# denix56/SI-Mamba

Hardware: AMD Instinct MI355X
Metric: point-clouds/sec (fwd+bwd) (higher is better)
Workload: dtype f32; 1 GPU; PointMamba classifier train step (FPS+kNN grouping, encoder, spectral SAST ordering, 12 Mamba blocks d=384 at L=1024, head, AdamW), 1024 pts -> 128 patches; global_batch=64, per_gpu_batch=64, npoints=1024, patches=128, mamba_seq_len=1024, parallelism=dp1, communicator_ranks=1, library_gemm=tuned solution table (si_mamba_amd/tuned/gemm_gfx950.csv)

## Files before the change

include/simamba.h:

```cpp
#ifndef SIMAMBA_H_
#define SIMAMBA_H_

#include <stddef.h>

#ifdef __cplusplus
extern "C" {
#endif

#define SIMAMBA_ABI_VERSION 9

#define SIMAMBA_F32  0
#define SIMAMBA_BF16 1

#define SIMAMBA_OK            0
#define SIMAMBA_E_NULLPTR    -1
#define SIMAMBA_E_SHAPE      -2
#define SIMAMBA_E_DTYPE      -3
#define SIMAMBA_E_DSTATE     -4
#define SIMAMBA_E_WIDTH      -5
#define SIMAMBA_E_WORKSPACE  -6
#define SIMAMBA_E_GROUPS     -7
#define SIMAMBA_E_ALIGN      -8
#define SIMAMBA_E_VARIANT    -9
#define SIMAMBA_E_BIAS       -10
// ... 60 lines not shown
                                  void* du, void* ddelta, float* dA, float* dB, float* dC, float* dD, void* dz,
                                  float* ddelta_bias, int batch, int dim, int seqlen, int dstate, int dt_rank,
                                  int io_dtype, long long z_bstride, long long dz_bstride, long long xdbl_bstride,
                                  long long xdbl_tstride, void* stream);
int simamba_selective_scan_dt_bwd_ex(const void* u, const void* xdbl, const void* wdt, const float* A, const float* D,
                                     const void* z, const float* delta_bias, const void* dout, const float* x_ckpt,
                                     void* du, void* ddelta, float* dA, float* dB, float* dC, float* dD, void* dz,
                                     float* ddelta_bias, int batch, int dim, int seqlen, int dstate, int dt_rank,
                                     int io_dtype, long long z_bstride, long long dz_bstride, long long xdbl_bstride,
                                     long long xdbl_tstride, int flags, float* workspace, long long workspace_floats,
                                     void* stream);

int simamba_xdt_proj_fwd(const void* x, const void* wx, const void* wdt, void* xdbl, void* delta,
                         int batch, int D, int seqlen, int S, int R, int io_dtype, long long x_bstride,
                         void* stream);
int simamba_conv_xdt_proj_fwd(const void* x, const float* cw, const float* cb, const void* wx, const void* wdt,
                              void* xconv, void* xdbl, void* delta, int batch, int D, int seqlen, int S, int R,
                              int io_dtype, long long x_bstride, void* stream);

int simamba_seq_gather_fwd(const void* in, const int* idx, void* out, int batch, int channels, int G, int L,
                           long long out_bstride, int io_dtype, void* stream);
int simamba_seq_gather_bwd(const void* dout, const int* inv, void* din, int batch, int channels, int G, int L,
                           int R, long long dout_bstride, int io_dtype, void* stream);

int simamba_causal_conv1d_fwd(const void* x, const float* w, const float* bias, void* out,
                              int batch, int dim, int seqlen, int width, int silu,
                              int io_dtype, long long x_bstride, void* stream);
int simamba_causal_conv1d_bwd(const void* x, const float* w, const float* bias,
                              const void* dout, void* dx, float* dw, float* dbias,
                              int batch, int dim, int seqlen, int width, int silu,
                              int io_dtype, long long x_bstride, long long dx_bstride, void* stream);
long long simamba_causal_conv1d_bwd_workspace_floats(int batch, int dim, int seqlen, int width, int flags);
int simamba_causal_conv1d_bwd_ex(const void* x, const float* w, const float* bias,
                                 const void* dout, void* dx, float* dw, float* dbias,
                                 int batch, int dim, int seqlen, int width, int silu,
                                 int io_dtype, long long x_bstride, long long dx_bstride, int flags,
                                 float* workspace, long long workspace_floats, void* stream);

int simamba_add_layer_norm_grid(int batch, int rows_per_batch);
int simamba_add_layer_norm_fwd(const void* hidden, const float* residual, const float* rowscale,
                               const float* weight, const float* bias, float* residual_out,
                               void* normed, float* mean, float* rstd, int batch, int rows_per_batch,
                               int dim, float eps, int hidden_dtype, int out_dtype, void* stream);
int simamba_add_layer_norm_bwd(const void* dnormed, const float* dresidual_out,
                               const float* residual_out, const float* mean, const float* rstd,
                               const float* weight, const float* rowscale, float* dresidual,
// ... 37 lines not shown
                           float eps, float* mean, float* invstd, double* count, int C, void* stream);
int simamba_bn_relu_apply(const void* x, const float* gterm, int group, const float* weight, const float* bias,
                          const float* mean, const float* invstd, void* y, long long rows, int C, long long ld,
                          int io_dtype, void* stream);
int simamba_bn_relu_bwd_sums(const void* dy, const void* x, const float* gterm, int group, const float* weight,
                             const float* bias, const float* mean, const float* invstd, float* dweight,
                             float* dbias, float* partial, long long rows, int C, long long ld, int io_dtype,
                             void* stream);
int simamba_bn_relu_bwd_dx(const void* dy, const void* x, const float* gterm, int group, const float* weight,
                           const float* bias, const float* mean, const float* invstd, const float* sum_dweight,
                           const float* sum_dbias, const double* count, void* dx, float* dgterm, int dgroup,
                           long long rows, int C, long long ld, int io_dtype, void* stream);
int simamba_group_max_fwd(const void* x, void* out, unsigned char* idx, long long groups, int n, int C,
                          int io_dtype, void* stream);
int simamba_group_max_bwd(const void* dout, const unsigned char* idx, void* dx, long long groups, int n, int C,
                          int io_dtype, void* stream);

int simamba_max_linear_bwd_slabs(long long groups, int c_in);
int simamba_max_linear_bwd_dx(const void* dout, const unsigned char* idx, const void* weight, void* dx,
                              long long groups, int n, int c_in, int c_out, int io_dtype, void* stream);
int simamba_max_linear_bwd_dw(const void* dout, const unsigned char* idx, const void* x, float* dw, float* partial,
                              long long groups, int n, int c_in, int c_out, int io_dtype, void* stream);

int simamba_three_nn(const float* xyz1, const float* xyz2, int* idx, float* weight, int batch, int N, int S,
                     void* stream);
int simamba_three_interpolate_fwd(const void* feats, const int* idx, const float* weight, void* out, int batch,
                                  int N, int S, int C, int io_dtype, void* stream);
int simamba_three_interpolate_bwd(const void* dout, const int* idx, const float* weight, float* dfeats, int batch,
                                  int N, int S, int C, int io_dtype, void* stream);

int simamba_chamfer_fwd(const float* pred, const float* gt, float* dist, unsigned char* idx1, unsigned char* idx2,
                        long long pairs, int n, int m, void* stream);
int simamba_chamfer_bwd(const float* pred, const float* gt, const float* ddist, const unsigned char* idx1,
                        const unsigned char* idx2, float* dpred, long long pairs, int n, int m, void* stream);

int simamba_chamfer_large_fwd(const float* x, const float* y, float* dist, int* idx1, int* idx2, float* d1, float* d2,
                              long long pairs, int n, int m, void* stream);
int simamba_chamfer_large_bwd(const float* x, const float* y, const float* ddist, const int* idx1, const int* idx2,
                              float* dx, float* dy, long long pairs, int n, int m, void* stream);
int simamba_chamfer_large_fwd_ex(const float* x, const float* y, float* dist, int* idx1, int* idx2, float* d1,
                                 float* d2, long long pairs, int n, int m, int queries, void* stream);
int simamba_chamfer_large_bwd_ex(const float* x, const float* y, const float* ddist, const int* idx1, const int* idx2,
                                 float* dx, float* dy, long long pairs, int n, int m, int queries, void* stream);

int simamba_knn_group(const float* points, const float* centers, long long* idx, int batch, int N, int G, int K,
                      void* stream);
// ... 41 lines not shown
```

si_mamba_amd/_lib.py:

```python
from __future__ import annotations

import ctypes
import os
from ctypes import c_char_p, c_float, c_int, c_longlong, c_size_t, c_uint, c_void_p

_HERE = os.path.dirname(os.path.abspath(__file__))
LIB_PATH = os.path.join(_HERE, "libsimamba_hip.so")

F32, BF16 = 0, 1

SPEC_SYMMETRIC = 0x01
SPEC_SELF_LOOP = 0x02
SPEC_BINARY = 0x04
SPEC_MATRIX_SYM = 0x08
SPEC_SMALLEST = 0x10
SPEC_SIGMA_MEAN = 0x20
SPEC_LARGE_G = 0x40
SPEC_MAX_G = 128
SPEC_MAX_G_LARGE = 512

SCAN_AUTO, SCAN_ROWSCAN, SCAN_LPC2, SCAN_LPC4, SCAN_MIX = 0, 1, 2, 4, 6
CKPT_ROW, CKPT_SEQ = 128, 16
BWD_DETERMINISTIC = 1
NORM_RMS = 1
# ... 18 lines not shown
                                           c_int, c_int, c_int, c_int, c_int, c_int,
                                           _LL, _LL, _LL, _LL, _LL, c_int, _P]),
    "simamba_scan_bwd_workspace_floats": (_LL, [c_int, c_int, c_int, c_int, c_int, c_int]),
    "simamba_selective_scan_bwd_ex": (c_int, [_P, _P, _P, _P, _P, _P, _P, _P, _P, _P,
                                              _P, _P, _P, _P, _P, _P, _P, _P,
                                              c_int, c_int, c_int, c_int, c_int, c_int,
                                              _LL, _LL, _LL, _LL, _LL, c_int, c_int, _P, _LL, _P]),
    "simamba_selective_scan_dt_fwd": (c_int, [_P, _P, _P, _P, _P, _P, _P, _P, _P, _P,
                                              c_int, c_int, c_int, c_int, c_int, c_int,
                                              _LL, _LL, _LL, c_int, c_int, _P]),
    "simamba_selective_scan_dt_bwd": (c_int, [_P, _P, _P, _P, _P, _P, _P, _P, _P,
                                              _P, _P, _P, _P, _P, _P, _P, _P,
                                              c_int, c_int, c_int, c_int, c_int, c_int,
                                              _LL, _LL, _LL, _LL, _P]),
    "simamba_selective_scan_dt_bwd_ex": (c_int, [_P, _P, _P, _P, _P, _P, _P, _P, _P,
                                                 _P, _P, _P, _P, _P, _P, _P, _P,
                                                 c_int, c_int, c_int, c_int, c_int, c_int,
                                                 _LL, _LL, _LL, _LL, c_int, _P, _LL, _P]),
    "simamba_xdt_proj_fwd": (c_int, [_P, _P, _P, _P, _P, c_int, c_int, c_int, c_int, c_int, c_int, _LL, _P]),
    "simamba_conv_xdt_proj_fwd": (c_int, [_P, _P, _P, _P, _P, _P, _P, _P, c_int, c_int, c_int, c_int, c_int, c_int, _LL,
                                          _P]),
    "simamba_seq_gather_fwd": (c_int, [_P, _P, _P, c_int, c_int, c_int, c_int, _LL, c_int, _P]),
    "simamba_seq_gather_bwd": (c_int, [_P, _P, _P, c_int, c_int, c_int, c_int, c_int, _LL, c_int, _P]),
    "simamba_causal_conv1d_fwd": (c_int, [_P, _P, _P, _P, c_int, c_int, c_int, c_int, c_int, c_int, _LL, _P]),
    "simamba_causal_conv1d_bwd": (c_int, [_P, _P, _P, _P, _P, _P, _P,
                                          c_int, c_int, c_int, c_int, c_int, c_int, _LL, _LL, _P]),
    "simamba_causal_conv1d_bwd_workspace_floats": (_LL, [c_int, c_int, c_int, c_int, c_int]),
    "simamba_causal_conv1d_bwd_ex": (c_int, [_P, _P, _P, _P, _P, _P, _P,
                                             c_int, c_int, c_int, c_int, c_int, c_int, _LL, _LL, c_int, _P, _LL, _P]),
    "simamba_add_layer_norm_grid": (c_int, [c_int, c_int]),
    "simamba_add_layer_norm_fwd": (c_int, [_P, _P, _P, _P, _P, _P, _P, _P, _P, c_int, c_int, c_int, c_float,
                                           c_int, c_int, _P]),
    "simamba_add_layer_norm_bwd": (c_int, [_P, _P, _P, _P, _P, _P, _P, _P, _P, _P, c_int, c_int, c_int,
                                           c_int, c_int, _P]),
    "simamba_add_layer_norm_fwd_ex": (c_int, [_P, _P, _P, _P, _P, _P, _P, _P, _P, c_int, c_int, c_int, c_float,
                                              c_int, c_int, c_int, _P]),
    "simamba_add_layer_norm_bwd_ex": (c_int, [_P, _P, _P, _P, _P, _P, _P, _P, _P, _P, c_int, c_int, c_int,
                                              c_int, c_int, c_int, _P]),
    "simamba_out_proj_add_ln_fwd": (c_int, [_P, _P, _P, _P, _P, _P, _P, _P, _P, _P, c_int, c_int, c_int, c_int, c_float,
                                            c_int, _P]),
    "simamba_out_proj_add_ln_fwd_ex": (c_int, [_P, _P, _P, _P, _P, _P, _P, _P, _P, _P, c_int, c_int, c_int, c_int,
                                               c_float, c_int, c_int, _P]),
    "simamba_in_proj_fwd": (c_int, [_P, _P, _P, c_int, c_int, c_int, c_int, c_int, _P]),
    "simamba_bn_relu_grid": (c_int, [_LL]),
    "simamba_bn_relu_fwd": (c_int, [_P, _P, c_int, _P, _P, _P, _P, c_float, c_float, c_int, _P, _P, _P, _P, _LL, c_int,
                                    _LL, c_int, _P]),
    "simamba_bn_relu_bwd": (c_int, [_P, _P, _P, c_int, _P, _P, _P, _P, _P, _P, c_int, _P, _P, _P, _LL, c_int, _LL,
                                    c_int, c_int, _P]),
    "simamba_bn_stats_local": (c_int, [_P, _P, c_int, _P, _LL, _P, _LL, c_int, _LL, c_int, _P]),
    "simamba_bn_stats_merge": (c_int, [_P, c_int, _P, _P, c_float, c_float, _P, _P, _P, c_int, _P]),
    "simamba_bn_relu_apply": (c_int, [_P, _P, c_int, _P, _P, _P, _P, _P, _LL, c_int, _LL, c_int, _P]),
    "simamba_bn_relu_bwd_sums": (c_int, [_P, _P, _P, c_int, _P, _P, _P, _P, _P, _P, _P, _LL, c_int, _LL, c_int, _P]),
    "simamba_bn_relu_bwd_dx": (c_int, [_P, _P, _P, c_int, _P, _P, _P, _P, _P, _P, _P, _P, _P, c_int, _LL, c_int, _LL,
                                       c_int, _P]),
    "simamba_group_max_fwd": (c_int, [_P, _P, _P, _LL, c_int, c_int, c_int, _P]),
    "simamba_group_max_bwd": (c_int, [_P, _P, _P, _LL, c_int, c_int, c_int, _P]),
    "simamba_max_linear_bwd_slabs": (c_int, [_LL, c_int]),
    "simamba_max_linear_bwd_dx": (c_int, [_P, _P, _P, _P, _LL, c_int, c_int, c_int, c_int, _P]),
    "simamba_max_linear_bwd_dw": (c_int, [_P, _P, _P, _P, _P, _LL, c_int, c_int, c_int, c_int, _P]),
    "simamba_three_nn": (c_int, [_P, _P, _P, _P, c_int, c_int, c_int, _P]),
    "simamba_three_interpolate_fwd": (c_int, [_P, _P, _P, _P, c_int, c_int, c_int, c_int, c_int, _P]),
    "simamba_three_interpolate_bwd": (c_int, [_P, _P, _P, _P, c_int, c_int, c_int, c_int, c_int, _P]),
    "simamba_chamfer_fwd": (c_int, [_P, _P, _P, _P, _P, _LL, c_int, c_int, _P]),
    "simamba_chamfer_bwd": (c_int, [_P, _P, _P, _P, _P, _P, _LL, c_int, c_int, _P]),
    "simamba_chamfer_large_fwd": (c_int, [_P, _P, _P, _P, _P, _P, _P, _LL, c_int, c_int, _P]),
    "simamba_chamfer_large_bwd": (c_int, [_P, _P, _P, _P, _P, _P, _P, _LL, c_int, c_int, _P]),
    "simamba_chamfer_large_fwd_ex": (c_int, [_P, _P, _P, _P, _P, _P, _P, _LL, c_int, c_int, c_int, _P]),
    "simamba_chamfer_large_bwd_ex": (c_int, [_P, _P, _P, _P, _P, _P, _P, _LL, c_int, c_int, c_int, _P]),
    "simamba_knn_group": (c_int, [_P, _P, _P, c_int, c_int, c_int, c_int, _P]),
    "simamba_knn_group_ex": (c_int, [_P, _P, _P, _P, _P, c_int, c_int, c_int, c_int, _P]),
    "simamba_knn_graph": (c_int, [_P, _P, _P, c_size_t, c_int, c_int, c_int, c_int, c_float, c_uint, _P]),
    "simamba_laplacian_topk": (c_int, [_P, _P, _P, _P, _P, _P, c_int, c_int, c_int, c_uint, _P]),
    "simamba_laplacian_topk_workspace_bytes": (c_size_t, [c_int, c_int]),
    "simamba_laplacian_topk_ex": (c_int, [_P, _P, _P, _P, _P, c_size_t, c_int, c_int, c_int, c_uint, _P]),
    "simamba_spectral_workspace_bytes": (c_size_t, [c_int, c_int]),
    "simamba_spectral_topk": (c_int, [_P, _P, _P, _P, _P, c_size_t, c_int, c_int, c_int, c_float,
                                      c_int, c_uint, _P]),
    "simamba_argsort_rows": (c_int, [_P, _P, c_int, c_int, _P]),
    "simamba_farthest_point_sample": (c_int, [_P, _P, _P, c_int, c_int, c_int, _P]),
    "simamba_farthest_point_sample_ex": (c_int, [_P, _P, _P, _P, _P, c_int, c_int, c_int, _P]),
}

# ... 169 lines not shown
_hand_in_proj = [None]


class fuse_out_norm(_Override):
    cell = _fuse_out_norm


def fuse_out_norm_enabled():
    return _fuse_out_norm[0]


_sparse_max_linear = [None]


class sparse_max_linear(_Override):
    cell, coerce = _sparse_max_linear, staticmethod(_tristate)


def sparse_max_linear_enabled(dtype):
    import torch
    return (dtype == torch.float32) if _sparse_max_linear[0] is None else _sparse_max_linear[0]


class hand_in_proj(_Override):
    cell, coerce = _hand_in_proj, staticmethod(_tristate)


def in_proj_hand_enabled(workgroups, dtype=None):
    import torch
    if _hand_in_proj[0] is not None:
        return _hand_in_proj[0]
    return dtype != torch.float32 and workgroups >= IN_PROJ_MIN_WORKGROUPS


IN_PROJ_MIN_WORKGROUPS = 192


def scan_plan_step(batch, dim, seqlen, dstate, dtype, *, softplus=True, has_z=True, act_addr_or=0, a_addr=0,
                   b_addr=0, c_addr=0, z_bs=0, dz_bs=0, bc_strides=(0, 0, 0)):
    lib = load()
    code = dtype_code(dtype)
    step = _scan_ckpt[0] or lib.simamba_scan_ckpt_step(batch, dim, seqlen, dstate, code)
    if step == CKPT_SEQ and not lib.simamba_scan_seq_applicable(
            batch, dim, seqlen, dstate, code, int(bool(softplus)), int(bool(has_z)), act_addr_or, a_addr, b_addr,
            c_addr, z_bs, dz_bs, *bc_strides):
        step = CKPT_ROW
# ... 64 lines not shown
```

si_mamba_amd/csrc/det_reduce.h:

```cpp
#pragma once
#include <hip/hip_runtime.h>

namespace simamba {

struct DetSumJob {
  const float* part;
  float* out;
  long long kstride;
  long long n;
  int K;
};

constexpr int kDetSumMaxJobs = 5;

int det_sum_launch(const DetSumJob* jobs, int njobs, hipStream_t s);

}
```

si_mamba_amd/csrc/det_reduce.hip:

```cpp
#include "det_reduce.h"

namespace simamba {

constexpr int kDetSumThreads = 256;
constexpr int kDetSumPerBlock = 4 * kDetSumThreads;

struct DetSumArgs {
  DetSumJob job[kDetSumMaxJobs];
  int vec[kDetSumMaxJobs];
  int blk0[kDetSumMaxJobs + 1];
  int njobs;
};

__global__ __launch_bounds__(kDetSumThreads) void det_sum_kernel(DetSumArgs a) {
  const int blk = blockIdx.x;
  int j = 0;
#pragma unroll
  for (int q = 1; q < kDetSumMaxJobs; ++q) j = (q < a.njobs && blk >= a.blk0[q]) ? q : j;
  const float* __restrict__ part = a.job[j].part;
  float* __restrict__ out = a.job[j].out;
  const long long ks = a.job[j].kstride, n = a.job[j].n;
  const int K = a.job[j].K;
  const long long i0 = (static_cast<long long>(blk - a.blk0[j]) * kDetSumThreads + threadIdx.x) * 4;
  if (i0 >= n) return;
  if (a.vec[j] && i0 + 4 <= n) {
    const float* p = part + i0;
    float4 acc = make_float4(0.f, 0.f, 0.f, 0.f);
    int k = 0;
    for (; k + 4 <= K; k += 4) {
      float4 v[4];
#pragma unroll
      for (int m = 0; m < 4; ++m) v[m] = *reinterpret_cast<const float4*>(p + (k + m) * ks);
#pragma unroll
      for (int m = 0; m < 4; ++m) {
        acc.x += v[m].x; acc.y += v[m].y; acc.z += v[m].z; acc.w += v[m].w;
      }
    }
    for (; k < K; ++k) {
      const float4 v = *reinterpret_cast<const float4*>(p + k * ks);
      acc.x += v.x; acc.y += v.y; acc.z += v.z; acc.w += v.w;
    }
    *reinterpret_cast<float4*>(out + i0) = acc;
    return;
  }
  for (long long i = i0; i < n && i < i0 + 4; ++i) {
    float acc = 0.f;
    for (int k = 0; k < K; ++k) acc += part[k * ks + i];
    out[i] = acc;
  }
}

int det_sum_launch(const DetSumJob* jobs, int njobs, hipStream_t s) {
  DetSumArgs a{};
  int blocks = 0, m = 0;
  for (int i = 0; i < njobs && m < kDetSumMaxJobs; ++i) {
    if (jobs[i].n <= 0) continue;
    a.job[m] = jobs[i];
    a.vec[m] = (reinterpret_cast<uintptr_t>(jobs[i].part) & 15u) == 0 && (reinterpret_cast<uintptr_t>(jobs[i].out) & 15u) == 0 &&
               jobs[i].kstride % 4 == 0;
    a.blk0[m] = blocks;
    blocks += static_cast<int>((jobs[i].n + kDetSumPerBlock - 1) / kDetSumPerBlock);
    ++m;
  }
  if (!m) return static_cast<int>(hipSuccess);
  a.njobs = m;
  for (int q = m; q <= kDetSumMaxJobs; ++q) a.blk0[q] = blocks;
  hipLaunchKernelGGL(det_sum_kernel, dim3(blocks), dim3(kDetSumThreads), 0, s, a);
  return static_cast<int>(hipGetLastError());
}

}
```

si_mamba_amd/csrc/encoder_sparse.hip:

```cpp
#include "det_reduce.h"
#include "host_common.h"

namespace simamba {

constexpr int kSpCols = 64;
constexpr int kSpWaves = 16;
constexpr int kSpThreads = kSpWaves * 64;
constexpr int kSpMaxN = 32;
constexpr int kSpMaxCout = 384;
constexpr int kSpChunks = kSpMaxCout / 64;
constexpr int kSpCpw = kSpMaxCout / kSpWaves;
constexpr int kSpTilePatches = 8;
constexpr int kSpTileRegs = kSpCpw / 8;
constexpr int kSpTileQuads = kSpTilePatches * kSpMaxN * (kSpCols / 4) / kSpThreads;
constexpr int kSpTargetWorkgroups = 256;
constexpr long long kSpMaxGroups = 1ll << 30;
constexpr int kSpDxMinSlab = kSpWaves;
static_assert(kSpTilePatches * 8 == 64 && kSpCpw % 8 == 0, "a register holds 8 channels of each of a tile's 8 patches");

template <typename T>
__device__ __forceinline__ float4 load_quad(const T* p) {
  const Pack<T, 4> pk = *reinterpret_cast<const Pack<T, 4>*>(p);
  return make_float4(to_f32<T>(pk.v[0]), to_f32<T>(pk.v[1]), to_f32<T>(pk.v[2]), to_f32<T>(pk.v[3]));
}
// ... 99 lines not shown
      if (e < tile_rows * (kSpCols / 4)) *reinterpret_cast<float4*>(tile + 4 * e) = xq[q];
    }
    int idc[kSpTileRegs];
    float dc[kSpTileRegs];
#pragma unroll
    for (int q = 0; q < kSpTileRegs; ++q) { idc[q] = id[q]; dc[q] = d[q]; }
    __syncthreads();
    if (g + kSpTilePatches < g1) fetch(g + kSpTilePatches);
    const float* xl = tile + lane;
#pragma unroll 1
    for (int p = 0; p < kSpTilePatches; ++p) {
#pragma unroll
      for (int j = 0; j < kSpCpw; ++j) {
        const int row = __builtin_amdgcn_readlane(idc[j / 8], p * 8 + j % 8);
        acc[j] = fmaf(read_lane(dc[j / 8], p * 8 + j % 8), xl[row * kSpCols], acc[j]);
      }
    }
    buf ^= 1;
  }
  float* out = partial + (static_cast<long long>(blockIdx.y) * cout + c0) * cin + col0 + lane;
#pragma unroll
  for (int j = 0; j < kSpCpw; ++j)
    if (j < cnt) out[static_cast<long long>(j) * cin] = acc[j];
}

constexpr int kSpDxLds = kSpMaxCout * kSpCols * 4;
constexpr int kSpDwLds = 2 * (kSpTilePatches * kSpMaxN + 1) * kSpCols * 4;

static int max_linear_check(int io_dtype, long long groups, int n, int cin, int cout, bool pointers, bool aligned) {
  if (const int rc = check_io_dtype(io_dtype)) return rc;
  if (groups == 0) return 1;
  if (groups < 0 || groups > kSpMaxGroups || n < 1 || n > kSpMaxN || cin < kSpCols || (cin % kSpCols) != 0 ||
      cin > 65536 || cout < 4 || (cout % 4) != 0 || cout > kSpMaxCout)
    return SIMAMBA_E_SHAPE;
  if (!pointers) return SIMAMBA_E_NULLPTR;
  if (!aligned) return SIMAMBA_E_ALIGN;
  return SIMAMBA_OK;
}

static int slab_of(long long groups, int cin, int floor) {
  const long long slabs = max(1ll, static_cast<long long>(kSpTargetWorkgroups / (cin / kSpCols)));
  return static_cast<int>(max(static_cast<long long>(floor), (groups + slabs - 1) / slabs));
}

}

// ... 26 lines not shown
extern "C" int simamba_max_linear_bwd_dw(const void* dout, const unsigned char* idx, const void* x, float* dw,
                                         float* partial, long long groups, int n, int c_in, int c_out, int io_dtype,
                                         void* stream) {
  if (const int rc = max_linear_check(io_dtype, groups, n, c_in, c_out, dout && idx && x && dw && partial,
                                      aligned16(dout) && aligned16(x) && aligned16(dw) && aligned16(partial)))
    return rc > 0 ? SIMAMBA_OK : rc;
  hipStream_t s = static_cast<hipStream_t>(stream);
  const int slab = slab_of(groups, c_in, kSpTilePatches);
  const int slabs = static_cast<int>((groups + slab - 1) / slab);
  const dim3 grid(c_in / kSpCols, slabs);
  const size_t lds = sizeof(float) * 2 * (kSpTilePatches * n + 1) * kSpCols;
  const int rc = with_io_type(io_dtype, [&](auto tag) {
    using T = decltype(tag);
    if (const hipError_t e = ensure_lds_cap<max_linear_bwd_dw_kernel<T>>(kSpDwLds)) return static_cast<int>(e);
    hipLaunchKernelGGL(max_linear_bwd_dw_kernel<T>, grid, dim3(kSpThreads), lds, s, static_cast<const T*>(dout), idx,
                       static_cast<const T*>(x), partial, groups, n, c_in, c_out, slab);
    return static_cast<int>(hipGetLastError());
  });
  if (rc) return rc;
  const long long elems = static_cast<long long>(c_out) * c_in;
  const DetSumJob job{partial, dw, elems, elems, slabs};
  return det_sum_launch(&job, 1, s);
}
```

si_mamba_amd/csrc/seq_gather.hip:

```cpp
#include "common.h"

namespace simamba {

constexpr int kSgThreads = 256;
constexpr int kSgMaxG = 256;
constexpr int kSgMaxL = 2048;

struct SgArgs {
  const void* in;
  void* out;
  const int* idx;
  int B, C, G, L, R;
  long long seq_bs;
};

template <typename T>
__global__ __launch_bounds__(kSgThreads) void seq_gather_fwd_kernel(SgArgs p) {
  __shared__ __attribute__((aligned(16))) float sRow[kSgThreads / 64][kSgMaxG];
  const int wave = threadIdx.x >> 6, lane = threadIdx.x & 63;
  const int b = blockIdx.y;
  const int G = p.G, L = p.L;
  constexpr int kMaxPacks = kSgMaxL / 4 / 64;
  const int npk = (L / 4 + 63) / 64;
  int tok[kMaxPacks][4];
// ... 111 lines not shown
  return static_cast<int>(hipGetLastError());
}

extern "C" int simamba_seq_gather_bwd(const void* dout, const int* inv, void* din, int batch, int channels, int G, int L,
                                      int R, long long dout_bstride, int io_dtype, void* stream) {
  if (int rc = sg_check(batch, channels, G, L, io_dtype)) return rc;
  if (R <= 0 || R > 8 || static_cast<long long>(G) * R != L) return SIMAMBA_E_SHAPE;
  if (batch == 0) return SIMAMBA_OK;
  if (!dout || !inv || !din) return SIMAMBA_E_NULLPTR;
  SgArgs a{};
  a.in = dout; a.out = din; a.idx = inv; a.B = batch; a.C = channels; a.G = G; a.L = L; a.R = R;
  a.seq_bs = dout_bstride ? dout_bstride : static_cast<long long>(channels) * L;
  const size_t esz = io_dtype == SIMAMBA_F32 ? 4 : 2;
  if (reinterpret_cast<uintptr_t>(dout) & (4 * esz - 1) || a.seq_bs % 4) return SIMAMBA_E_ALIGN;
  int gx = (channels + 3) / 4;
  while (gx > 1 && static_cast<long long>(gx) * batch > 4096) gx = (gx + 1) / 2;
  dim3 grid(gx, batch);
  if (io_dtype == SIMAMBA_F32)
    hipLaunchKernelGGL(seq_gather_bwd_kernel<float>, grid, dim3(kSgThreads), 0, static_cast<hipStream_t>(stream), a);
  else
    hipLaunchKernelGGL(seq_gather_bwd_kernel<bf16_t>, grid, dim3(kSgThreads), 0, static_cast<hipStream_t>(stream), a);
  return static_cast<int>(hipGetLastError());
}
```

si_mamba_amd/encoder_ops.py:

```python
from __future__ import annotations

import torch
import torch.distributed as dist

from . import _lib


_BN_MAX_C = 1024
_BN_CHUNK = 256


_SPLITK = 64
_SPLITK_MIN_ROWS = 512


class TokenLinearFn(torch.autograd.Function):

    @staticmethod
    def forward(ctx, x, weight, bias):
        y = torch.nn.functional.linear(x, weight, bias)
        ctx.save_for_backward(x, weight)
        ctx.has_bias = bias is not None
        return y

# ... 284 lines not shown
        out = torch.empty(groups, C, device=dev, dtype=xc.dtype)
        idx = torch.empty(groups, C, device=dev, dtype=torch.uint8)
        with torch.cuda.device(dev):
            _abi("simamba_group_max_fwd", xc.data_ptr(), out.data_ptr(), idx.data_ptr(), groups, n, C, code,
                 _lib.stream_ptr(dev))
        ctx.save_for_backward(idx)
        ctx.meta = (groups, n, C, code, xc.dtype)
        return out

    @staticmethod
    def backward(ctx, dout):
        (idx,) = ctx.saved_tensors
        groups, n, C, code, dtype = ctx.meta
        d = dout.to(dtype).contiguous()
        dx = torch.empty(groups, n, C, device=d.device, dtype=dtype)
        with torch.cuda.device(d.device):
            _abi("simamba_group_max_bwd", d.data_ptr(), idx.data_ptr(), dx.data_ptr(), groups, n, C, code,
                 _lib.stream_ptr(d.device))
        return dx


def group_max_fn(x):
    return GroupMaxFn.apply(x)


_SPARSE_MAX_N = 32
_SPARSE_MAX_COUT = 384


def _linear_io_dtype(x):
    return torch.get_autocast_dtype("cuda") if (x.is_cuda and torch.is_autocast_enabled("cuda")) else x.dtype


def token_linear_group_max_ok(x, weight, n):
    if not (x.is_cuda and x.dim() == 2 and weight.dim() == 2 and _lib.sparse_max_linear_enabled(_linear_io_dtype(x))):
        return False
    rows, cin = x.shape
    cout = weight.shape[0]
    return (1 <= n <= _SPARSE_MAX_N and rows > 0 and rows % n == 0 and cin == weight.shape[1] and cin % 64 == 0
            and cout % 4 == 0 and 4 <= cout <= _SPARSE_MAX_COUT
            and _linear_io_dtype(x) in (torch.float32, torch.bfloat16)
            and x.is_contiguous() and x.data_ptr() % 16 == 0)


class TokenLinearGroupMaxFn(torch.autograd.Function):

# ... 53 lines not shown
```

si_mamba_amd/mamba_inner.py:

```python
from __future__ import annotations

import torch

from . import _lib


def _w(t, dtype):
    return t if t.dtype == dtype else t.to(dtype)


def _wx(W, X):
    return torch.bmm(W.unsqueeze(0).expand(X.shape[0], -1, -1), X)


def _xw(X, W):
    return torch.bmm(X, W.unsqueeze(0).expand(X.shape[0], -1, -1))


def _sum_bmm(X, Y):
    return torch.bmm(X, Y).sum(0, dtype=torch.float32)


class InProjFn(torch.autograd.Function):

    @staticmethod
    def forward(ctx, hidden, weight, bias):
        io = hidden.dtype
        if torch.is_autocast_enabled("cuda"):
            io = torch.get_autocast_dtype("cuda")
            hidden = hidden.to(io)
        wc = _w(weight, io)
        xz = tokens_times_weight(hidden, wc) if bias is None else _wx(wc, hidden.transpose(1, 2))
        if bias is not None:
            xz = xz + _w(bias, io)[None, :, None]
        ctx.save_for_backward(hidden, weight)
        ctx.wc = wc
        ctx.has_bias = bias is not None
        return xz

    @staticmethod
    def backward(ctx, dxz):
        hidden, weight = ctx.saved_tensors
        io = hidden.dtype
# ... 154 lines not shown
                            None if D is None else D.dtype, None if delta_bias is None else delta_bias.dtype)
        ctx.save_for_backward(xz, x_conv, x_dbl, delta, None if no_out else y, cw, cb, x_proj_w, dt_proj_w, out_proj_w,
                              Af, Df, bf, x_ckpt)
        return out

    @staticmethod
    def backward(ctx, dout):
        (xz, x_conv, x_dbl, delta, y, cw, cb, x_proj_w, dt_proj_w, out_proj_w, Af, Df, bf, x_ckpt) = ctx.saved_tensors
        lib = _lib.load()
        R, N, W = ctx.dims
        io = xz.dtype
        code = _lib.dtype_code(io)
        Bsz, twoD, L = xz.shape
        Dm = twoD // 2
        S = R + 2 * N
        dev = xz.device
        stream = _lib.stream_ptr(dev)
        xbs = xz.stride(0)
        dout = dout.to(io)
        f32 = dict(device=dev, dtype=torch.float32)
        xw_c, dtw_c, ow_c = ctx.wcast
        if ctx.no_out:
            dy = dout.contiguous()
            d_out_w = d_out_b = None
        else:
            if dout.stride(2) != 1:
                dout = dout.contiguous()
            d_out_w = _sum_bmm(dout.transpose(1, 2), y.transpose(1, 2))
            d_out_b = dout.sum((0, 1)) if ctx.has_out_bias else None
            dy = tokens_times_weight(dout, ow_c.t())

        dxz = torch.empty_like(xz)
        du = torch.empty(Bsz, Dm, L, device=dev, dtype=io)
        ddelta = torch.empty(Bsz, Dm, L, device=dev, dtype=io)
        dA, dB, dC, dD, dbias = _lib.scan_bwd_accumulators(Bsz, Dm, L, N, Df is not None, bf is not None, dev)
        Bv, Cv = x_dbl[:, :, R:R + N], x_dbl[:, :, R + N:]
        z, dz = xz[:, Dm:], dxz[:, Dm:]
        flags, ws, nws = _lib.det_args(lib.simamba_scan_bwd_workspace_floats, Bsz, Dm, L, N,
                                       _lib.CKPT_SEQ if ctx.dtw_k is not None else ctx.ckpt_step, device=dev)
        _lib.count("scan_bwd_det" if flags else "scan_bwd_atomic")
        with torch.cuda.device(dev), _lib.timed("scan_bwd", dev):
            if ctx.dtw_k is not None:
                rc = lib.simamba_selective_scan_dt_bwd_ex(
                    x_conv.data_ptr(), x_dbl.data_ptr(), ctx.dtw_k.data_ptr(), Af.data_ptr(), _lib.ptr(Df),
                    z.data_ptr(), _lib.ptr(bf), dy.data_ptr(), _lib.ptr(x_ckpt),
                    du.data_ptr(), ddelta.data_ptr(), dA.data_ptr(), dB.data_ptr(), dC.data_ptr(), _lib.ptr(dD),
                    dz.data_ptr(), _lib.ptr(dbias), Bsz, Dm, L, N, R, code,
                    xbs, dxz.stride(0), x_dbl.stride(0), x_dbl.stride(1), flags, _lib.ptr(ws), nws, stream)
            else:
                rc = lib.simamba_selective_scan_bwd_ex(
                    x_conv.data_ptr(), delta.data_ptr(), Af.data_ptr(), Bv.data_ptr(), Cv.data_ptr(), _lib.ptr(Df),
                    z.data_ptr(), _lib.ptr(bf), dy.data_ptr(), _lib.ptr(x_ckpt),
                    du.data_ptr(), ddelta.data_ptr(), dA.data_ptr(), dB.data_ptr(), dC.data_ptr(), _lib.ptr(dD),
                    dz.data_ptr(), _lib.ptr(dbias), Bsz, Dm, L, N, code, 1,
                    xbs, dxz.stride(0), x_dbl.stride(0), 1, x_dbl.stride(1), ctx.ckpt_step, flags, _lib.ptr(ws), nws,
                    stream)
        _lib.check(rc, "simamba_selective_scan_bwd_ex")

        dx_dbl = torch.empty(Bsz, L, S, device=dev, dtype=io)
        dx_dbl[:, :, :R].copy_(_xw(ddelta.transpose(1, 2), dtw_c))
        dBC = torch.as_strided(dB, (2, Bsz, N, L), (Bsz * N * L, N * L, L, 1))
        dx_dbl[:, :, R:].view(Bsz, L, 2, N).copy_(dBC.permute(1, 3, 0, 2))
        d_dt_w = _sum_bmm(ddelta, x_dbl[:, :, :R])
        d_x_w = _sum_bmm(dx_dbl.transpose(1, 2), x_conv.transpose(1, 2))
        wxT = xw_c.t().unsqueeze(0).expand(Bsz, -1, -1)
        torch.baddbmm(du, wxT, dx_dbl.transpose(1, 2), out=du)

        dconv = torch.empty(Dm * W + (Dm if cb is not None else 0), **f32)
        dcw = dconv[:Dm * W].view(Dm, W)
        dcb = dconv[Dm * W:] if cb is not None else None
        flags, ws, nws = _lib.det_args(lib.simamba_causal_conv1d_bwd_workspace_floats, Bsz, Dm, L, W, device=dev)
        _lib.count("conv1d_bwd_det" if flags else "conv1d_bwd_atomic")
        with torch.cuda.device(dev), _lib.timed("conv1d_bwd", dev):
            rc = lib.simamba_causal_conv1d_bwd_ex(xz.data_ptr(), cw.data_ptr(), _lib.ptr(cb), du.data_ptr(),
                                                  dxz.data_ptr(), dcw.data_ptr(), _lib.ptr(dcb),
                                                  Bsz, Dm, L, W, 1, code, xbs, dxz.stride(0), flags, _lib.ptr(ws), nws,
                                                  stream)
        _lib.check(rc, "simamba_causal_conv1d_bwd_ex")

        t_cw, t_cb, t_xw, t_dtw, t_ow, t_A, t_D, t_b = ctx.param_dtypes
        return (dxz, dcw.to(t_cw), None if dcb is None else dcb.to(t_cb), d_x_w.to(t_xw), d_dt_w.to(t_dtw),
                None if d_out_w is None else d_out_w.to(t_ow),
                None if d_out_b is None else d_out_b.to(out_proj_w.dtype), dA.to(t_A),
                None if dD is None else dD.to(t_D), None if dbias is None else dbias.to(t_b), None, None, None)


def mamba_inner_fn(xz, conv1d_weight, conv1d_bias, x_proj_weight, delta_proj_weight, out_proj_weight,
                   out_proj_bias, A, D=None, delta_bias=None, dt_rank=None, d_state=None):
    if conv1d_weight.dim() == 3:
        conv1d_weight = conv1d_weight.squeeze(1)
    if dt_rank is None:
        dt_rank = delta_proj_weight.shape[1]
    if d_state is None:
        d_state = (x_proj_weight.shape[0] - dt_rank) // 2
    return MambaInnerFn.apply(xz, conv1d_weight, conv1d_bias, x_proj_weight, delta_proj_weight, out_proj_weight,
                              out_proj_bias, A, D, delta_bias, dt_rank, d_state, torch.is_grad_enabled())
```

si_mamba_amd/point_mamba.py:

```python
from __future__ import annotations

from types import SimpleNamespace

import torch
import torch.nn as nn

from . import grouping, spectral
from .block import MixerModel
from .add_norm import add_layer_norm_fn
from .encoder_ops import bn_relu_fn, group_max_fn, token_linear, token_linear_group_max


class Group(nn.Module):

    def __init__(self, num_group, group_size):
        super().__init__()
        self.num_group = num_group
        self.group_size = group_size
        self.fps_fn = grouping.sample_farthest_points

    @torch.no_grad()
    def _indices(self, xyz, lengths=None):
        if lengths is not None:
            if not (xyz.is_cuda and xyz.shape[1] <= 8192):
                raise NotImplementedError("Group: lengths are taken by the HIP kernels only (a ROCm device, clouds of "
                                          "up to 8192 points)")
            need = max(self.num_group, self.group_size)
            if not torch.cuda.is_current_stream_capturing():
                shortest = int(lengths.min())
                if shortest < need:
                    raise ValueError(f"Group: the shortest cloud has {shortest} points, every cloud needs at least "
                                     f"{need} (max of num_group = {self.num_group} and group_size = {self.group_size})")
            center, _ = self.fps_fn(xyz, self.num_group, lengths=lengths)
# ... 15 lines not shown

class Encoder(nn.Module):

    def __init__(self, encoder_channel):
        super().__init__()
        self.encoder_channel = encoder_channel
        self.fused = True
        self.first_conv = nn.Sequential(nn.Conv1d(3, 128, 1), nn.BatchNorm1d(128), nn.ReLU(inplace=True),
                                        nn.Conv1d(128, 256, 1))
        self.second_conv = nn.Sequential(nn.Conv1d(512, 512, 1), nn.BatchNorm1d(512), nn.ReLU(inplace=True),
                                         nn.Conv1d(512, self.encoder_channel, 1))

    def forward(self, point_groups):
        bs, g, n, _ = point_groups.shape
        c1, bn1, _, c2 = self.first_conv
        c3, bn2, _, c4 = self.second_conv
        lin = torch.nn.functional.linear
        x = point_groups.reshape(bs * g * n, 3)
        if self.fused and x.is_cuda and 256 % n == 0:
            lin = token_linear
            x = bn_relu_fn(lin(x, c1.weight.squeeze(-1), c1.bias), bn1)
            f = lin(x, c2.weight.squeeze(-1), c2.bias)
            cf = f.shape[1]
            fg = group_max_fn(f.view(bs * g, n, cf))
            w3 = c3.weight.squeeze(-1)
            gterm = lin(fg, w3[:, :cf], c3.bias)
            x = bn_relu_fn(lin(f, w3[:, cf:]), bn2, gterm=gterm, group=n)
            return token_linear_group_max(x, c4.weight.squeeze(-1), c4.bias, n).reshape(bs, g, self.encoder_channel)
        x = torch.relu(bn1(lin(x, c1.weight.squeeze(-1), c1.bias)))
        f = lin(x, c2.weight.squeeze(-1), c2.bias).view(bs * g, n, 256)
        fg = f.max(dim=1, keepdim=True)[0]
        x = torch.cat([fg.expand(-1, n, -1), f], dim=2).reshape(bs * g * n, 512)
        x = torch.relu(bn2(lin(x, c3.weight.squeeze(-1), c3.bias)))
        f = lin(x, c4.weight.squeeze(-1), c4.bias).view(bs * g, n, self.encoder_channel)
        return f.max(dim=1)[0].reshape(bs, g, self.encoder_channel)


def default_config(**over):
    cfg = dict(trans_dim=384, depth=12, cls_dim=15, group_size=32, num_group=128, encoder_dims=384,
               rms_norm=False, drop_path=0.1, drop_out=0., method="SAST", reverse=True, knn_graph=20,
               k_top_eigenvectors=4, alpha=10., smallest=True, symmetric=True, self_loop=False,
               binary=True, matrix="laplacian")
    cfg.update(over)
    return SimpleNamespace(**cfg)


def plackett_luce_dist(logits):
# ... 138 lines not shown
```

Baseline: 1135 point-clouds/s.

## Fuse Mamba backward weight-gradient sums, xdbl packing, and group-max gradient scatter

Adds a batched multi-job reduction kernel with split accumulators that sums the per-batch bmm weight-gradient partials of out_proj, dt_proj and x_proj in one launch. A new pack kernel builds dx_dbl from d_dt, dB and dC through shared memory, replacing two strided copies. In the encoder, the group-max gradient is scatter-added in place into the dense gradient instead of materialising a separate tensor and adding it. The aim is fewer launches and less memory traffic in backward, at the cost of more custom kernels and non-atomic in-place scatter semantics.

Result: no change. 1142 point-clouds/s, median of 6 (+0.6%).

```diff
diff --git a/include/simamba.h b/include/simamba.h
--- a/include/simamba.h
+++ b/include/simamba.h
@@ -106,6 +106,9 @@
                            long long out_bstride, int io_dtype, void* stream);
 int simamba_seq_gather_bwd(const void* dout, const int* inv, void* din, int batch, int channels, int G, int L,
                            int R, long long dout_bstride, int io_dtype, void* stream);
+
+int simamba_xdbl_pack(const void* prod, const float* dB, const float* dC, void* out, int batch, int seqlen, int R,
+                      int N, int io_dtype, void* stream);
 
 int simamba_causal_conv1d_fwd(const void* x, const float* w, const float* bias, void* out,
                               int batch, int dim, int seqlen, int width, int silu,
@@ -189,6 +192,12 @@
 int simamba_max_linear_bwd_dw(const void* dout, const unsigned char* idx, const void* x, float* dw, float* partial,
                               long long groups, int n, int c_in, int c_out, int io_dtype, void* stream);
 
+int simamba_group_max_scatter_add(const void* dmax, const unsigned char* idx, void* dense, long long groups, int n,
+                                  int C, int io_dtype, void* stream);
+
+int simamba_batch_sum(const float* const* partials, const int* K, const long long* kstride, const long long* n,
+                      float* const* out, int njobs, void* stream);
+
 int simamba_three_nn(const float* xyz1, const float* xyz2, int* idx, float* weight, int batch, int N, int S,
                      void* stream);
 int simamba_three_interpolate_fwd(const void* feats, const int* idx, const float* weight, void* out, int batch,
diff --git a/si_mamba_amd/_lib.py b/si_mamba_amd/_lib.py
--- a/si_mamba_amd/_lib.py
+++ b/si_mamba_amd/_lib.py
@@ -64,6 +64,7 @@
                                           _P]),
     "simamba_seq_gather_fwd": (c_int, [_P, _P, _P, c_int, c_int, c_int, c_int, _LL, c_int, _P]),
     "simamba_seq_gather_bwd": (c_int, [_P, _P, _P, c_int, c_int, c_int, c_int, c_int, _LL, c_int, _P]),
+    "simamba_xdbl_pack": (c_int, [_P, _P, _P, _P, c_int, c_int, c_int, c_int, c_int, _P]),
     "simamba_causal_conv1d_fwd": (c_int, [_P, _P, _P, _P, c_int, c_int, c_int, c_int, c_int, c_int, _LL, _P]),
     "simamba_causal_conv1d_bwd": (c_int, [_P, _P, _P, _P, _P, _P, _P,
                                           c_int, c_int, c_int, c_int, c_int, c_int, _LL, _LL, _P]),
@@ -100,6 +101,8 @@
     "simamba_max_linear_bwd_slabs": (c_int, [_LL, c_int]),
     "simamba_max_linear_bwd_dx": (c_int, [_P, _P, _P, _P, _LL, c_int, c_int, c_int, c_int, _P]),
     "simamba_max_linear_bwd_dw": (c_int, [_P, _P, _P, _P, _P, _LL, c_int, c_int, c_int, c_int, _P]),
+    "simamba_group_max_scatter_add": (c_int, [_P, _P, _P, _LL, c_int, c_int, c_int, _P]),
+    "simamba_batch_sum": (c_int, [_P, _P, _P, _P, _P, c_int, _P]),
     "simamba_three_nn": (c_int, [_P, _P, _P, _P, c_int, c_int, c_int, _P]),
     "simamba_three_interpolate_fwd": (c_int, [_P, _P, _P, _P, c_int, c_int, c_int, c_int, c_int, _P]),
     "simamba_three_interpolate_bwd": (c_int, [_P, _P, _P, _P, c_int, c_int, c_int, c_int, c_int, _P]),
@@ -315,6 +318,45 @@
     return (dtype == torch.float32) if _sparse_max_linear[0] is None else _sparse_max_linear[0]
 
 
+_backward_passes = [True]
+pass_counters = {}
+
+
+def count_pass(name):
+    pass_counters[name] = pass_counters.get(name, 0) + 1
+
+
+class backward_passes(_Override):
+    cell = _backward_passes
+
+
+def backward_passes_enabled():
+    return _backward_passes[0]
+
+
+def batch_sum(partials):
+    import torch
+    n = len(partials)
+    outs = [torch.empty(p.shape[1:], device=p.device, dtype=torch.float32) for p in partials]
+    arr_p = (c_void_p * n)(*[p.data_ptr() for p in partials])
+    arr_o = (c_void_p * n)(*[o.data_ptr() for o in outs])
+    arr_k = (c_int * n)(*[p.shape[0] for p in partials])
+    numel = [o.numel() for o in outs]
+    arr_n = (c_longlong * n)(*numel)
+    dev = partials[0].device
+    with torch.cuda.device(dev):
+        rc = load().simamba_batch_sum(arr_p, arr_k, arr_n, arr_n, arr_o, n, stream_ptr(dev))
+    check(rc, "simamba_batch_sum")
+    return outs
+
+
+def batch_sum_ok(*partials):
+    import torch
+    return backward_passes_enabled() and all(
+        p.is_cuda and p.dtype == torch.float32 and p.dim() >= 2 and p.is_contiguous() and p.numel() > 0
+        for p in partials)
+
+
 class hand_in_proj(_Override):
     cell, coerce = _hand_in_proj, staticmethod(_tristate)
 
diff --git a/si_mamba_amd/csrc/det_reduce.h b/si_mamba_amd/csrc/det_reduce.h
--- a/si_mamba_amd/csrc/det_reduce.h
+++ b/si_mamba_amd/csrc/det_reduce.h
@@ -13,6 +13,6 @@
 
 constexpr int kDetSumMaxJobs = 5;
 
-int det_sum_launch(const DetSumJob* jobs, int njobs, hipStream_t s);
+int det_sum_launch(const DetSumJob* jobs, int njobs, hipStream_t s, bool split = false);
 
 }
diff --git a/si_mamba_amd/csrc/det_reduce.hip b/si_mamba_amd/csrc/det_reduce.hip
--- a/si_mamba_amd/csrc/det_reduce.hip
+++ b/si_mamba_amd/csrc/det_reduce.hip
@@ -1,10 +1,10 @@
 #include "det_reduce.h"
+#include "host_common.h"
 
 namespace simamba {
 
 constexpr int kDetSumThreads = 256;
 constexpr int kDetSumPerBlock = 4 * kDetSumThreads;
-
 struct DetSumArgs {
   DetSumJob job[kDetSumMaxJobs];
   int vec[kDetSumMaxJobs];
@@ -12,7 +12,8 @@
   int njobs;
 };
 
-__global__ __launch_bounds__(kDetSumThreads) void det_sum_kernel(DetSumArgs a) {
+template <int kU, bool kSplit>
+__device__ __forceinline__ void det_sum_body(const DetSumArgs& a) {
   const int blk = blockIdx.x;
   int j = 0;
 #pragma unroll
@@ -23,34 +24,60 @@
   const int K = a.job[j].K;
   const long long i0 = (static_cast<long long>(blk - a.blk0[j]) * kDetSumThreads + threadIdx.x) * 4;
   if (i0 >= n) return;
+  constexpr int kAcc = kSplit ? kU : 1;
   if (a.vec[j] && i0 + 4 <= n) {
     const float* p = part + i0;
-    float4 acc = make_float4(0.f, 0.f, 0.f, 0.f);
+    float4 acc[kAcc];
+#pragma unroll
+    for (int m = 0; m < kAcc; ++m) acc[m] = make_float4(0.f, 0.f, 0.f, 0.f);
     int k = 0;
-    for (; k + 4 <= K; k += 4) {
-      float4 v[4];
+    for (; k + kU <= K; k += kU) {
+      float4 v[kU];
 #pragma unroll
-      for (int m = 0; m < 4; ++m) v[m] = *reinterpret_cast<const float4*>(p + (k + m) * ks);
+      for (int m = 0; m < kU; ++m) v[m] = *reinterpret_cast<const float4*>(p + (k + m) * ks);
 #pragma unroll
-      for (int m = 0; m < 4; ++m) {
-        acc.x += v[m].x; acc.y += v[m].y; acc.z += v[m].z; acc.w += v[m].w;
+      for (int m = 0; m < kU; ++m) {
+        float4& s = acc[kSplit ? m : 0];
+        s.x += v[m].x; s.y += v[m].y; s.z += v[m].z; s.w += v[m].w;
       }
     }
-    for (; k < K; ++k) {
-      const float4 v = *reinterpret_cast<const float4*>(p + k * ks);
-      acc.x += v.x; acc.y += v.y; acc.z += v.z; acc.w += v.w;
+#pragma unroll
+    for (int m = 0; m < kU - 1; ++m) {
+      if (k + m < K) {
+        const float4 v = *reinterpret_cast<const float4*>(p + (k + m) * ks);
+        float4& s = acc[kSplit ? m : 0];
+        s.x += v.x; s.y += v.y; s.z += v.z; s.w += v.w;
+      }
     }
-    *reinterpret_cast<float4*>(out + i0) = acc;
+#pragma unroll
+    for (int h = kAcc / 2; h > 0; h /= 2)
+#pragma unroll
+      for (int m = 0; m < h; ++m) {
+        acc[m].x += acc[m + h].x; acc[m].y += acc[m + h].y; acc[m].z += acc[m + h].z; acc[m].w += acc[m + h].w;
+      }
+    *reinterpret_cast<float4*>(out + i0) = acc[0];
     return;
   }
   for (long long i = i0; i < n && i < i0 + 4; ++i) {
-    float acc = 0.f;
-    for (int k = 0; k < K; ++k) acc += part[k * ks + i];
-    out[i] = acc;
+    float acc[kAcc];
+#pragma unroll
+    for (int m = 0; m < kAcc; ++m) acc[m] = 0.f;
+    for (int k = 0; k < K; k += kAcc)
+#pragma unroll
+      for (int m = 0; m < kAcc; ++m)
+        if (k + m < K) acc[m] += part[(k + m) * ks + i];
+#pragma unroll
+    for (int h = kAcc / 2; h > 0; h /= 2)
+#pragma unroll
+      for (int m = 0; m < h; ++m) acc[m] += acc[m + h];
+    out[i] = acc[0];
   }
 }
 
-int det_sum_launch(const DetSumJob* jobs, int njobs, hipStream_t s) {
+__global__ __launch_bounds__(kDetSumThreads) void det_sum_kernel(DetSumArgs a) { det_sum_body<4, false>(a); }
+__global__ __launch_bounds__(kDetSumThreads) void batch_sum_kernel(DetSumArgs a) { det_sum_body<8, true>(a); }
+
+int det_sum_launch(const DetSumJob* jobs, int njobs, hipStream_t s, bool split) {
   DetSumArgs a{};
   int blocks = 0, m = 0;
   for (int i = 0; i < njobs && m < kDetSumMaxJobs; ++i) {
@@ -65,8 +92,33 @@
   if (!m) return static_cast<int>(hipSuccess);
   a.njobs = m;
   for (int q = m; q <= kDetSumMaxJobs; ++q) a.blk0[q] = blocks;
-  hipLaunchKernelGGL(det_sum_kernel, dim3(blocks), dim3(kDetSumThreads), 0, s, a);
+  if (split)
+    hipLaunchKernelGGL(batch_sum_kernel, dim3(blocks), dim3(kDetSumThreads), 0, s, a);
+  else
+    hipLaunchKernelGGL(det_sum_kernel, dim3(blocks), dim3(kDetSumThreads), 0, s, a);
   return static_cast<int>(hipGetLastError());
 }
 
 }
+
+using namespace simamba;
+
+extern "C" int simamba_batch_sum(const float* const* partials, const int* K, const long long* kstride,
+                                 const long long* n, float* const* out, int njobs, void* stream) {
+  if (njobs < 0 || njobs > kDetSumMaxJobs) return SIMAMBA_E_SHAPE;
+  if (njobs == 0) return SIMAMBA_OK;
+  if (!partials || !K || !kstride || !n || !out) return SIMAMBA_E_NULLPTR;
+  DetSumJob jobs[kDetSumMaxJobs];
+  long long blocks = 0;
+  for (int j = 0; j < njobs; ++j) {
+    if (K[j] < 0 || n[j] < 0 || kstride[j] < 0 || (kstride[j] != 0 && kstride[j] < n[j]) || n[j] > (1ll << 40))
+      return SIMAMBA_E_SHAPE;
+    blocks += (n[j] + kDetSumPerBlock - 1) / kDetSumPerBlock;
+  }
+  if (blocks > 0x7fffffffll) return SIMAMBA_E_SHAPE;
+  for (int j = 0; j < njobs; ++j) {
+    if (n[j] > 0 && (!out[j] || (K[j] > 0 && !partials[j]))) return SIMAMBA_E_NULLPTR;
+    jobs[j] = DetSumJob{partials[j], out[j], kstride[j], n[j], K[j]};
+  }
+  return det_sum_launch(jobs, njobs, static_cast<hipStream_t>(stream), true);
+}
diff --git a/si_mamba_amd/csrc/encoder_sparse.hip b/si_mamba_amd/csrc/encoder_sparse.hip
--- a/si_mamba_amd/csrc/encoder_sparse.hip
+++ b/si_mamba_amd/csrc/encoder_sparse.hip
@@ -145,6 +145,23 @@
 #pragma unroll
   for (int j = 0; j < kSpCpw; ++j)
     if (j < cnt) out[static_cast<long long>(j) * cin] = acc[j];
+}
+
+
+constexpr int kSaThreads = 256;
+
+template <typename T>
+__global__ __launch_bounds__(kSaThreads) void group_max_scatter_add_kernel(
+    const T* __restrict__ dmax, const unsigned char* __restrict__ idx, T* __restrict__ dense, long long total, int n,
+    int C) {
+  const long long e = static_cast<long long>(blockIdx.x) * kSaThreads + threadIdx.x;
+  if (e >= total) return;
+  const int r = idx[e];
+  if (r >= n) return;
+  const long long g = e / C;
+  const int c = static_cast<int>(e - g * C);
+  T* at = dense + (g * n + r) * C + c;
+  *at = from_f32<T>(to_f32<T>(*at) + to_f32<T>(dmax[e]));
 }
 
 constexpr int kSpDxLds = kSpMaxCout * kSpCols * 4;
@@ -217,3 +234,21 @@
   const DetSumJob job{partial, dw, elems, elems, slabs};
   return det_sum_launch(&job, 1, s);
 }
+
+extern "C" int simamba_group_max_scatter_add(const void* dmax, const unsigned char* idx, void* dense, long long groups,
+                                             int n, int C, int io_dtype, void* stream) {
+  if (const int rc = check_io_dtype(io_dtype)) return rc;
+  if (groups < 0 || groups > kSpMaxGroups || n < 1 || n > kSpMaxN || C < 1 || C > 65536) return SIMAMBA_E_SHAPE;
+  if (groups == 0) return SIMAMBA_OK;
+  if (!dmax || !idx || !dense) return SIMAMBA_E_NULLPTR;
+  const long long total = groups * C;
+  const long long blocks = (total + kSaThreads - 1) / kSaThreads;
+  if (blocks > 0x7fffffffll) return SIMAMBA_E_SHAPE;
+  with_io_type(io_dtype, [&](auto tag) {
+    using T = decltype(tag);
+    hipLaunchKernelGGL(group_max_scatter_add_kernel<T>, dim3(static_cast<unsigned>(blocks)), dim3(kSaThreads), 0,
+                       static_cast<hipStream_t>(stream), static_cast<const T*>(dmax), idx, static_cast<T*>(dense), total,
+                       n, C);
+  });
+  return static_cast<int>(hipGetLastError());
+}
diff --git a/si_mamba_amd/csrc/seq_gather.hip b/si_mamba_amd/csrc/seq_gather.hip
--- a/si_mamba_amd/csrc/seq_gather.hip
+++ b/si_mamba_amd/csrc/seq_gather.hip
@@ -157,3 +157,52 @@
     hipLaunchKernelGGL(seq_gather_bwd_kernel<bf16_t>, grid, dim3(kSgThreads), 0, static_cast<hipStream_t>(stream), a);
   return static_cast<int>(hipGetLastError());
 }
+
+namespace simamba {
+
+constexpr int kXpTokens = 64;
+constexpr int kXpThreads = 256;
+constexpr int kXpMaxS = 128;
+
+__global__ __launch_bounds__(kXpThreads) void xdbl_pack_kernel(const float* __restrict__ prod,
+                                                               const float* __restrict__ dB,
+                                                               const float* __restrict__ dC, float* __restrict__ out,
+                                                               int L, int R, int N) {
+  __shared__ __attribute__((aligned(16))) float tile[kXpTokens * kXpMaxS];
+  const int S = R + 2 * N;
+  const int b = blockIdx.y;
+  const int l0 = blockIdx.x * kXpTokens;
+  const int rows = min(kXpTokens, L - l0);
+  const long long tok0 = static_cast<long long>(b) * L + l0;
+  const float* src = prod + tok0 * R;
+  for (int e = threadIdx.x; e < rows * R; e += kXpThreads) tile[(e / R) * S + e % R] = src[e];
+  for (int e = threadIdx.x; e < 2 * N * kXpTokens; e += kXpThreads) {
+    const int row = e / kXpTokens, l = e % kXpTokens;
+    const float* acc = row < N ? dB : dC;
+    const int n = row < N ? row : row - N;
+    if (l < rows) tile[l * S + R + row] = acc[(static_cast<long long>(b) * N + n) * L + l0 + l];
+  }
+  __syncthreads();
+  float* dst = out + tok0 * S;
+  const int cnt = rows * S;
+  const int quads = (reinterpret_cast<uintptr_t>(dst) & 15u) == 0 ? cnt / 4 : 0;
+  for (int q = threadIdx.x; q < quads; q += kXpThreads)
+    *reinterpret_cast<float4*>(dst + 4 * q) = *reinterpret_cast<const float4*>(tile + 4 * q);
+  for (int e = 4 * quads + threadIdx.x; e < cnt; e += kXpThreads) dst[e] = tile[e];
+}
+
+}
+
+extern "C" int simamba_xdbl_pack(const void* prod, const float* dB, const float* dC, void* out, int batch, int seqlen,
+                                 int R, int N, int io_dtype, void* stream) {
+  if (io_dtype != SIMAMBA_F32) return SIMAMBA_E_DTYPE;
+  if (batch < 0 || batch > 65535 || seqlen <= 0 || R < 0 || N < 1 || R + 2 * N > kXpMaxS ||
+      static_cast<long long>(seqlen) + kXpTokens > 0x7fffffffll)
+    return SIMAMBA_E_SHAPE;
+  if (batch == 0) return SIMAMBA_OK;
+  if ((R > 0 && !prod) || !dB || !dC || !out) return SIMAMBA_E_NULLPTR;
+  const dim3 grid((seqlen + kXpTokens - 1) / kXpTokens, batch);
+  hipLaunchKernelGGL(xdbl_pack_kernel, grid, dim3(kXpThreads), 0, static_cast<hipStream_t>(stream),
+                     static_cast<const float*>(prod), dB, dC, static_cast<float*>(out), seqlen, R, N);
+  return static_cast<int>(hipGetLastError());
+}
diff --git a/si_mamba_amd/encoder_ops.py b/si_mamba_amd/encoder_ops.py
--- a/si_mamba_amd/encoder_ops.py
+++ b/si_mamba_amd/encoder_ops.py
@@ -330,6 +330,55 @@
 
 def group_max_fn(x):
     return GroupMaxFn.apply(x)
+
+
+class GroupMaxKeepFn(torch.autograd.Function):
+
+    @staticmethod
+    def forward(ctx, x, n):
+        rows, C = x.shape
+        groups = rows // n
+        dev = x.device
+        code = _lib.dtype_code(x.dtype)
+        out = torch.empty(groups, C, device=dev, dtype=x.dtype)
+        idx = torch.empty(groups, C, device=dev, dtype=torch.uint8)
+        with torch.cuda.device(dev):
+            _abi("simamba_group_max_fwd", x.data_ptr(), out.data_ptr(), idx.data_ptr(), groups, n, C, code,
+                 _lib.stream_ptr(dev))
+        ctx.save_for_backward(idx)
+        ctx.meta = (groups, int(n), C, code, x.dtype)
+        ctx.set_materialize_grads(False)
+        return x, out
+
+    @staticmethod
+    def backward(ctx, dx, dmax):
+        (idx,) = ctx.saved_tensors
+        groups, n, C, code, dtype = ctx.meta
+        if dmax is None:
+            return dx, None
+        d = dmax.to(dtype).contiguous()
+        dev = d.device
+        st = _lib.stream_ptr(dev)
+        with torch.cuda.device(dev):
+            if dx is not None and dx.dtype == dtype and dx.is_contiguous():
+                _abi("simamba_group_max_scatter_add", d.data_ptr(), idx.data_ptr(), dx.data_ptr(), groups, n, C, code, st)
+                return dx, None
+            dm = torch.empty(groups * n, C, device=dev, dtype=dtype)
+            _abi("simamba_group_max_bwd", d.data_ptr(), idx.data_ptr(), dm.data_ptr(), groups, n, C, code, st)
+        return (dm if dx is None else dx + dm), None
+
+
+def group_max_keep_ok(x, n):
+    return (_lib.backward_passes_enabled() and x.is_cuda and x.dtype == torch.float32 and x.dim() == 2
+            and x.is_contiguous() and 1 <= n <= _SPARSE_MAX_N and x.shape[0] > 0 and x.shape[0] % n == 0
+            and x.shape[1] % 4 == 0)
+
+
+def group_max_keep(x, n):
+    if group_max_keep_ok(x, n):
+        _lib.count_pass("group_max_keep")
+        return GroupMaxKeepFn.apply(x, n)
+    return x, group_max_fn(x.view(x.shape[0] // n, n, x.shape[1]))
 
 
 _SPARSE_MAX_N = 32
diff --git a/si_mamba_amd/mamba_inner.py b/si_mamba_amd/mamba_inner.py
--- a/si_mamba_amd/mamba_inner.py
+++ b/si_mamba_amd/mamba_inner.py
@@ -19,6 +19,16 @@
 
 def _sum_bmm(X, Y):
     return torch.bmm(X, Y).sum(0, dtype=torch.float32)
+
+
+def _batch_sums(parts):
+    live = [p for p in parts if p is not None]
+    if live and len(live) <= 5 and _lib.batch_sum_ok(*live):
+        _lib.count_pass("batch_sum")
+        sums = iter(_lib.batch_sum(live))
+    else:
+        sums = iter([p.sum(0, dtype=torch.float32) for p in live])
+    return [None if p is None else next(sums) for p in parts]
 
 
 class InProjFn(torch.autograd.Function):
@@ -219,11 +229,11 @@
         xw_c, dtw_c, ow_c = ctx.wcast
         if ctx.no_out:
             dy = dout.contiguous()
-            d_out_w = d_out_b = None
+            p_out_w = d_out_b = None
         else:
             if dout.stride(2) != 1:
                 dout = dout.contiguous()
-            d_out_w = _sum_bmm(dout.transpose(1, 2), y.transpose(1, 2))
+            p_out_w = torch.bmm(dout.transpose(1, 2), y.transpose(1, 2))
             d_out_b = dout.sum((0, 1)) if ctx.has_out_bias else None
             dy = tokens_times_weight(dout, ow_c.t())
 
@@ -255,11 +265,22 @@
         _lib.check(rc, "simamba_selective_scan_bwd_ex")
 
         dx_dbl = torch.empty(Bsz, L, S, device=dev, dtype=io)
-        dx_dbl[:, :, :R].copy_(_xw(ddelta.transpose(1, 2), dtw_c))
-        dBC = torch.as_strided(dB, (2, Bsz, N, L), (Bsz * N * L, N * L, L, 1))
-        dx_dbl[:, :, R:].view(Bsz, L, 2, N).copy_(dBC.permute(1, 3, 0, 2))
-        d_dt_w = _sum_bmm(ddelta, x_dbl[:, :, :R])
-        d_x_w = _sum_bmm(dx_dbl.transpose(1, 2), x_conv.transpose(1, 2))
+        d_dt = _xw(ddelta.transpose(1, 2), dtw_c)
+        if xdbl_pack_ok(d_dt, dB, dC, S):
+            _lib.count_pass("xdbl_pack")
+            with torch.cuda.device(dev):
+                rc = lib.simamba_xdbl_pack(d_dt.data_ptr(), dB.data_ptr(), dC.data_ptr(), dx_dbl.data_ptr(), Bsz, L, R,
+                                           N, code, stream)
+            _lib.check(rc, "simamba_xdbl_pack")
+        else:
+            dx_dbl[:, :, :R].copy_(d_dt)
+            dBC = torch.as_strided(dB, (2, Bsz, N, L), (Bsz * N * L, N * L, L, 1))
+            dx_dbl[:, :, R:].view(Bsz, L, 2, N).copy_(dBC.permute(1, 3, 0, 2))
+        del d_dt
+        d_out_w, d_dt_w, d_x_w = _batch_sums([p_out_w,
+                                              torch.bmm(ddelta, x_dbl[:, :, :R]),
+                                              torch.bmm(dx_dbl.transpose(1, 2), x_conv.transpose(1, 2))])
+        del p_out_w
         wxT = xw_c.t().unsqueeze(0).expand(Bsz, -1, -1)
         torch.baddbmm(du, wxT, dx_dbl.transpose(1, 2), out=du)
 
@@ -282,6 +303,11 @@
                 None if dD is None else dD.to(t_D), None if dbias is None else dbias.to(t_b), None, None, None)
 
 
+def xdbl_pack_ok(d_dt, dB, dC, S):
+    return (_lib.backward_passes_enabled() and d_dt.dtype == torch.float32 and d_dt.is_contiguous()
+            and dB.is_contiguous() and dC.is_contiguous() and S <= 128 and d_dt.shape[0] <= 65535)
+
+
 def mamba_inner_fn(xz, conv1d_weight, conv1d_bias, x_proj_weight, delta_proj_weight, out_proj_weight,
                    out_proj_bias, A, D=None, delta_bias=None, dt_rank=None, d_state=None):
     if conv1d_weight.dim() == 3:
diff --git a/si_mamba_amd/point_mamba.py b/si_mamba_amd/point_mamba.py
--- a/si_mamba_amd/point_mamba.py
+++ b/si_mamba_amd/point_mamba.py
@@ -8,7 +8,7 @@
 from . import grouping, spectral
 from .block import MixerModel
 from .add_norm import add_layer_norm_fn
-from .encoder_ops import bn_relu_fn, group_max_fn, token_linear, token_linear_group_max
+from .encoder_ops import bn_relu_fn, group_max_keep, token_linear, token_linear_group_max
 
 
 class Group(nn.Module):
@@ -70,7 +70,7 @@
             x = bn_relu_fn(lin(x, c1.weight.squeeze(-1), c1.bias), bn1)
             f = lin(x, c2.weight.squeeze(-1), c2.bias)
             cf = f.shape[1]
-            fg = group_max_fn(f.view(bs * g, n, cf))
+            f, fg = group_max_keep(f, n)
             w3 = c3.weight.squeeze(-1)
             gterm = lin(fg, w3[:, :cf], c3.bias)
             x = bn_relu_fn(lin(f, w3[:, cf:]), bn2, gterm=gterm, group=n)
```
